# lrjconan/LanczosNetwork

Measured on NVIDIA H100. Metric: QM8 molecules/sec (forward), higher is better.
Workload: dtype f32

## Files before the change

### lanczosnetwork_b200/csrc/filter_mlp_chain.cu

```cuda
#include "tc_gemm.cuh"

namespace {

constexpr int S0MAX = 8;

struct ChainPolicy {
  static constexpr int kStagesB = 2;
  static constexpr int kStagesA = 4;
  struct Params {
    const float* table;
    const int32_t* rowmap;
    const int32_t* nrows;
    const float* W_hi;
    const float* W_lo;
    const float* bias_all;
    float* coeff;
    int Rall, L, S, Hd;
    int dbg;
  };
  static __device__ __forceinline__ bool mma0(const Params& p) { return p.S > S0MAX; }
  static __device__ __forceinline__ int first_stage(const Params& p) { return mma0(p) ? 0 : 1; }
  static __device__ __forceinline__ int steps_per_item(const Params& p) { return mma0(p) ? 4 : 2; }
  static __device__ __forceinline__ int rows(const Params& p) { return p.nrows ? __ldg(p.nrows) : p.Rall; }
  static __device__ __forceinline__ int ntile(const Params& p) { return (rows(p) + tcg::BM - 1) / tcg::BM; }
  static __device__ __forceinline__ void item_range(const Params& p, int cta, int ncta, int& first,
                                                    int& count) {
    const int items = ntile(p) * p.L, base = items / ncta, rem = items % ncta;
    count = base + (cta < rem ? 1 : 0);
    first = cta * base + min(cta, rem);
  }
  static __device__ __forceinline__ int num_steps(const Params& p, int cta, int ncta) {
    int first, count;
    item_range(p, cta, ncta, first, count);
    return count * steps_per_item(p);
  }
  static __device__ __forceinline__ void decode(const Params& p, int cta, int ncta, int it,
                                                int& m_tile, int& sub) {
    const int per = steps_per_item(p), nt = ntile(p);
    int first, count;
    item_range(p, cta, ncta, first, count);
    const int item = first + it / per;
    m_tile = item % nt;
    sub = (item / nt) * 4 + first_stage(p) + it % per;
  }
  static __device__ __forceinline__ int num_kblocks(const Params& p, int sub) {
    return (sub & 3) == 0 ? 1 : p.Hd / tcg::BK;
  }
  static __device__ __forceinline__ int w_row0(const Params& p, int layer, int stage) {
    return layer * (3 * p.Hd + p.S) + stage * p.Hd;
  }
  static __device__ __forceinline__ void w_coords(const Params& p, int sub, int kb, int& col0, int& row0) {
    col0 = kb * tcg::BK;
    row0 = w_row0(p, sub >> 2, sub & 3);
  }
  static __device__ __forceinline__ bool operand_from_acc(const Params& p, int sub) {
    return (sub & 3) > first_stage(p);
  }
  static __device__ __forceinline__ float acc_operand(const Params&, const uint8_t* policy_smem, int sub, int col,
                                                      float x) {
    const float* bs = reinterpret_cast<const float*>(policy_smem) + BS_OFF;
    return fmaxf(x + bs[(sub & 3) * tcg::BN + col], 0.f);
  }

  const Params& p;
  const int tid, r;
  static constexpr int BS_OFF = 2 * tcg::BN * S0MAX;
  float* W1s;
  float* W3s;
  float* bs;
  float* b3s;
  int src, cur_layer;
  float tv[S0MAX];
  float o[S0MAX];

  static size_t smem_bytes() {
    return (BS_OFF + 3 * tcg::BN + S0MAX) * 4;
  }

  __device__ ChainPolicy(const Params& p_, uint8_t* smem, int tid_)
      : p(p_), tid(tid_), r(tid_ & 127), src(-1), cur_layer(-1) {
    W1s = reinterpret_cast<float*>(smem);
    W3s = W1s + tcg::BN * S0MAX;
    bs = W1s + BS_OFF;
    b3s = bs + 3 * tcg::BN;
  }

  __device__ void step_begin(int m_tile, int sub, int, tcg::PhaseTimer& tm) {
    const int layer = sub >> 2;
    if ((sub & 3) != first_stage(p)) return;
    const int i = m_tile * tcg::BM + r;
    src = i < rows(p) ? (p.rowmap ? __ldg(p.rowmap + i) : i) : -1;
    if (layer != cur_layer) {
      tcg::producers_sync<ChainPolicy>();
      const int row0 = w_row0(p, layer, 0), row3 = w_row0(p, layer, 3);
      if (!mma0(p)) {
#pragma unroll 4
        for (int e = tid; e < p.Hd * S0MAX; e += tcg::producer_threads<ChainPolicy>) {
          const int c = e / S0MAX, k = e - c * S0MAX;
          const int64_t o1 = (int64_t)(row0 + c) * p.Hd + k;
          W1s[e] = (k < p.S) ? __ldg(p.W_hi + o1) + __ldg(p.W_lo + o1) : 0.f;
          const int64_t o3 = (int64_t)(row3 + k) * p.Hd + c;
          W3s[e] = (k < p.S) ? __ldg(p.W_hi + o3) + __ldg(p.W_lo + o3) : 0.f;
        }
        if (tid < S0MAX) b3s[tid] = tid < p.S ? __ldg(p.bias_all + row3 + tid) : 0.f;
      }
      for (int e = tid; e < 3 * tcg::BN; e += tcg::producer_threads<ChainPolicy>) {
        const int st = e / tcg::BN, c = e - st * tcg::BN;
        bs[e] = c < p.Hd ? __ldg(p.bias_all + row0 + st * p.Hd + c) : 0.f;
      }
      tcg::producers_sync<ChainPolicy>();
      cur_layer = layer;
      tm.lap(1);
    }
    if (mma0(p)) return;
#pragma unroll
    for (int k = 0; k < S0MAX; ++k)
      tv[k] = (src >= 0 && k < p.S) ? __ldg(p.table + (int64_t)src * p.S + k) : 0.f;
  }

  __device__ __forceinline__ void produce(int sub, int kb, float (&v)[32]) {
    if ((sub & 3) == 0) {
#pragma unroll
      for (int j = 0; j < 32; ++j)
        v[j] = (src >= 0 && j < p.S) ? __ldg(p.table + (int64_t)src * p.S + j) : 0.f;
      return;
    }
#pragma unroll
    for (int j = 0; j < 32; ++j) {
      const int c = kb * tcg::BK + j;
      const float4* wr = reinterpret_cast<const float4*>(W1s + c * S0MAX);
      const float4 wa = wr[0], wb = wr[1];
      float a = bs[c];
      a = fmaf(tv[0], wa.x, a); a = fmaf(tv[1], wa.y, a); a = fmaf(tv[2], wa.z, a); a = fmaf(tv[3], wa.w, a);
      a = fmaf(tv[4], wb.x, a); a = fmaf(tv[5], wb.y, a); a = fmaf(tv[6], wb.z, a); a = fmaf(tv[7], wb.w, a);
      v[j] = fmaxf(a, 0.f);
    }
  }
  __device__ __forceinline__ void pre_epilogue(int) {}
  __device__ __forceinline__ void post_epilogue(int) {}

  __device__ __forceinline__ void store(int sub, int col, const float (&x)[tcg::EW]) {
    const int layer = sub >> 2, stage = sub & 3;
    if (stage == 3) {
      if (src < 0 || col >= p.S) return;
      const float* bias = p.bias_all + w_row0(p, layer, stage);
      float* dst = p.coeff + ((int64_t)layer * p.Rall + src) * p.S;
#pragma unroll
      for (int j = 0; j < tcg::EW; ++j)
        if (col + j < p.S) dst[col + j] = x[j] + __ldg(bias + col + j);
      return;
    }
    if (col >= p.Hd) return;
    const float* b2 = bs + 2 * tcg::BN;
    if (col == 0) {
#pragma unroll
      for (int s = 0; s < S0MAX; ++s) o[s] = 0.f;
    }
#pragma unroll
    for (int j = 0; j < tcg::EW; ++j) {
      const float y = fmaxf(x[j] + b2[col + j], 0.f);
      const float4* wr = reinterpret_cast<const float4*>(W3s + (col + j) * S0MAX);
      const float4 wa = wr[0], wb = wr[1];
      o[0] = fmaf(y, wa.x, o[0]); o[1] = fmaf(y, wa.y, o[1]);
      o[2] = fmaf(y, wa.z, o[2]); o[3] = fmaf(y, wa.w, o[3]);
      o[4] = fmaf(y, wb.x, o[4]); o[5] = fmaf(y, wb.y, o[5]);
      o[6] = fmaf(y, wb.z, o[6]); o[7] = fmaf(y, wb.w, o[7]);
    }
    if (col + tcg::EW < p.Hd || src < 0) return;
    float* dst = p.coeff + ((int64_t)layer * p.Rall + src) * p.S;
#pragma unroll
    for (int s = 0; s < S0MAX; ++s)
      if (s < p.S) dst[s] = o[s] + b3s[s];
  }
};

__global__ void __launch_bounds__(1024)
ritz_rowmap_kernel(const int32_t* __restrict__ gext, int B, int K, int32_t* __restrict__ rowmap,
                   int32_t* __restrict__ nrows) {
  __shared__ int warp_sums[32];
  __shared__ int gbase[1024], gk[1024];
  __shared__ int running;
  const int tid = threadIdx.x, lane = tid & 31, warp = tid >> 5;
  if (tid == 0) running = 0;
  __syncthreads();
  for (int b0 = 0; b0 < B; b0 += 1024) {
    const int b = b0 + tid;
    int k = (b < B) ? min(gext[b * 2 + 1], K) : 0;
    int incl = k;
#pragma unroll
    for (int o = 1; o < 32; o <<= 1) {
      const int t = __shfl_up_sync(0xffffffffu, incl, o);
      if (lane >= o) incl += t;
    }
    if (lane == 31) warp_sums[warp] = incl;
    __syncthreads();
    if (warp == 0) {
      int w = warp_sums[lane], wi = w;
#pragma unroll
      for (int o = 1; o < 32; o <<= 1) {
        const int t = __shfl_up_sync(0xffffffffu, wi, o);
        if (lane >= o) wi += t;
      }
      warp_sums[lane] = wi - w;
    }
    __syncthreads();
    const int base = running + warp_sums[warp] + incl - k;
    gbase[tid] = base;
    gk[tid] = k;
    __syncthreads();
    if (tid == 1023) running = base + k;
    for (int j = warp; j < 1024 && b0 + j < B; j += 32)
      for (int i = lane; i < gk[j]; i += 32) rowmap[gbase[j] + i] = (b0 + j) * K + i;
    __syncthreads();
  }
  if (tid == 0) nrows[0] = running;
}

}

extern "C" {

int lnb_ritz_rowmap(lnb_stream_t stream, const int32_t* gext, int B, int K, int32_t* rowmap,
                    int32_t* nrows) {
  LNB_REQUIRE(gext && rowmap && nrows, "ritz_rowmap: null pointer");
  LNB_REQUIRE(B >= 0 && K >= 1, "ritz_rowmap: bad dims");
  ritz_rowmap_kernel<<<1, 1024, 0, (cudaStream_t)stream>>>(gext, B, K, rowmap, nrows);
  lnb::count_launch();
  return lnb::finish_launch("ritz_rowmap");
}

int lnb_ritz_filter_mlp(lnb_stream_t stream, const float* table, const int32_t* rowmap,
                        const int32_t* nrows, const float* W_hi, const float* W_lo,
                        const float* bias_all, int Rall, int L, int S, int Hd, float* coeff) {
  return lnb_ritz_filter_mlp_ctas(stream, table, rowmap, nrows, W_hi, W_lo, bias_all, Rall, L, S, Hd,
                                  coeff, 0);
}

int lnb_ritz_filter_mlp_ctas(lnb_stream_t stream, const float* table, const int32_t* rowmap,
                             const int32_t* nrows, const float* W_hi, const float* W_lo,
                             const float* bias_all, int Rall, int L, int S, int Hd, float* coeff,
                             int ctas) {
  LNB_REQUIRE(table && W_hi && W_lo && bias_all && coeff, "ritz_filter_mlp: null pointer");
  LNB_REQUIRE((rowmap == nullptr) == (nrows == nullptr), "ritz_filter_mlp: rowmap and nrows go together");
  LNB_REQUIRE(Rall >= 0 && L >= 1 && S >= 1 && Hd >= 1 && ctas >= 0, "ritz_filter_mlp: bad dims");
  if (S > 32 || Hd % 32 != 0 || Hd > tcg::BN) {
    lnb::set_err("ritz_filter_mlp: unsupported shape S=%d hidden=%d (needs S<=32, hidden%%32==0, hidden<=128)", S, Hd);
    return LNB_ERR_UNSUPPORTED;
  }
  if (Rall == 0) return LNB_OK;
  const size_t smem = tcg::core_smem(ChainPolicy::kStagesB, ChainPolicy::kStagesA) + 1024 + ChainPolicy::smem_bytes();
  ChainPolicy::Params p{table, rowmap, nrows, W_hi, W_lo, bias_all, coeff, Rall, L, S, Hd, tcg::debug_flags()};
  return tcg::launch<ChainPolicy>(stream, W_hi, W_lo, L * (3 * Hd + S), Hd, smem, lnb::ceil_div(Rall, tcg::BM) * L, p,
                                  "ritz_filter_mlp", ctas);
}

}
```

### lanczosnetwork_b200/csrc/tc_gemm.cuh

```cuda
#pragma once
#include "common.cuh"
#include "sm90.cuh"
#include <stdlib.h>
#include <type_traits>
#include <utility>

namespace tcg {

constexpr int BM = 128, BN = 128, BK = 32;
constexpr int TILE_B_BYTES = BN * BK * 4;
constexpr int STAGE_B_BYTES = 2 * TILE_B_BYTES;
constexpr int TILE_A_BYTES = BM * BK * 4;
constexpr int STAGE_A_BYTES = 2 * TILE_A_BYTES;
constexpr int EW = 16;
constexpr int CONSUMER_THREADS = 256;
constexpr int CONSUMER_REGS = 168;
constexpr int MAX_B_STAGES = 6, MAX_A_STAGES = 4;

template <class P, class = void> struct ProducerGroups : std::integral_constant<int, 1> {};
template <class P>
struct ProducerGroups<P, std::void_t<decltype(P::kProducerGroups)>> : std::integral_constant<int, P::kProducerGroups> {};
template <class P> constexpr int producer_threads = 128 * ProducerGroups<P>::value;
template <class P> constexpr int cta_threads = producer_threads<P> + CONSUMER_THREADS;
template <class P> constexpr int producer_regs = (65536 - CONSUMER_THREADS * CONSUMER_REGS) / producer_threads<P> / 8 * 8;
__host__ __device__ constexpr int core_smem(int stages_b, int stages_a) {
  return stages_b * STAGE_B_BYTES + stages_a * STAGE_A_BYTES + 256;
}
__host__ __device__ constexpr int pass_cols(int stages_a) {
  return stages_a * STAGE_A_BYTES / (BM * 4) < BN ? stages_a * STAGE_A_BYTES / (BM * 4) : BN;
}

__device__ __forceinline__ uint8_t* a_ring(uint8_t* policy_smem, int stages_b, int stages_a) {
  return policy_smem - core_smem(stages_b, stages_a) + stages_b * STAGE_B_BYTES;
}

struct Core {
  uint8_t* Bst;
  uint8_t* Ast;
  uint64_t* b_full;
  uint64_t* b_empty;
  uint64_t* a_full;
  uint64_t* a_empty;
  uint64_t* stg_full;
  uint64_t* stg_empty;
  uint64_t* kept_read;
};

__device__ __forceinline__ Core carve(uint8_t* base, int stages_b, int stages_a) {
  Core c;
  c.Bst = base;
  c.Ast = base + stages_b * STAGE_B_BYTES;
  uint64_t* bars = reinterpret_cast<uint64_t*>(c.Ast + stages_a * STAGE_A_BYTES);
  c.b_full = bars;
  c.b_empty = c.b_full + MAX_B_STAGES;
  c.a_full = c.b_empty + MAX_B_STAGES;
  c.a_empty = c.a_full + MAX_A_STAGES;
  c.stg_full = c.a_empty + MAX_A_STAGES;
  c.stg_empty = c.stg_full + 1;
  c.kept_read = c.stg_empty + 1;
  return c;
}

__device__ unsigned long long* g_prof = nullptr;

struct PhaseTimer {
  unsigned long long* buf;
  long long t0;
  __device__ __forceinline__ void start(int cta, int tid) {
    buf = (tid == 0 && g_prof) ? g_prof + cta * 32 : nullptr;
    if (buf) t0 = clock64();
  }
  __device__ __forceinline__ void start_if(int cta, bool owner) {
    buf = (owner && g_prof) ? g_prof + cta * 32 : nullptr;
    if (buf) t0 = clock64();
  }
  __device__ __forceinline__ void lap(int slot) {
    if (buf) { long long t = clock64(); atomicAdd(&buf[slot], (unsigned long long)(t - t0)); t0 = t; }
  }
};

template <class Policy>
__device__ __forceinline__ void producers_sync() {
  asm volatile("bar.sync 1, %0;" ::"n"(producer_threads<Policy>) : "memory");
}
__device__ __forceinline__ void consumers_sync() {
  asm volatile("bar.sync 2, %0;" ::"n"(CONSUMER_THREADS) : "memory");
}

__device__ __forceinline__ int stg_index(int row, int col, int pw) {
  return row * pw + ((((col >> 2) ^ row) & (pw / 4 - 1)) << 2) + (col & 3);
}

template <class P, class = void> struct HasAccInit : std::false_type {};
template <class P> struct HasAccInit<P, std::void_t<decltype(&P::acc_init)>> : std::true_type {};
template <class P, class = void> struct HasOperandFromAcc : std::false_type {};
template <class P> struct HasOperandFromAcc<P, std::void_t<decltype(&P::operand_from_acc)>> : std::true_type {};
template <class P>
constexpr bool kScaledProduce =
    std::is_same_v<decltype(std::declval<P&>().produce(0, 0, std::declval<float (&)[32]>())), float>;

template <class Policy>
__device__ __forceinline__ bool next_from_acc(const typename Policy::Params& p, int cta, int ncta, int it,
                                              int nsteps, int& nkb_next) {
  if (it + 1 >= nsteps) return false;
  int m_tile, sub;
  Policy::decode(p, cta, ncta, it + 1, m_tile, sub);
  nkb_next = Policy::num_kblocks(p, sub);
  return Policy::operand_from_acc(p, sub);
}

constexpr int SKIP_MMA = 2;
constexpr int SKIP_TMA = 4;

template <class Policy, int kSkip>
__device__ __forceinline__ void tc_gemm_body(const CUtensorMap& map_hi, const CUtensorMap& map_lo,
                                             const typename Policy::Params& p) {
  extern __shared__ __align__(16) uint8_t smem_raw[];
  const uint32_t pad = (1024u - (sm90::smem_u32(smem_raw) & 1023u)) & 1023u;
  uint8_t* base = smem_raw + pad;
  constexpr int SB = Policy::kStagesB, SA = Policy::kStagesA;
  static_assert(SB >= 1 && SB <= MAX_B_STAGES && SA >= 1 && SA <= MAX_A_STAGES, "ring depths");
  constexpr int PW = pass_cols(SA);
  constexpr int NPASS = BN / PW;
  constexpr bool kAccInit = HasAccInit<Policy>::value;
  static_assert(!kAccInit || NPASS == 1, "a drain kept in the A ring must fit it in one pass");
  constexpr bool kOpAcc = HasOperandFromAcc<Policy>::value;
  constexpr bool kQueue = !kAccInit;
  static_assert(!kOpAcc || SA * BK >= BN, "an operand written from the accumulators needs one A stage per k-block");
  constexpr int NG = ProducerGroups<Policy>::value, PT = producer_threads<Policy>;
  constexpr bool kScaled = kScaledProduce<Policy>;
  static_assert(NG == 1 || (NG == 2 && !kOpAcc && PW % (2 * EW) == 0), "two producer groups: no operand_from_acc");
  Core c = carve(base, SB, SA);
  uint8_t* policy_smem = base + core_smem(SB, SA);
  float* stg = reinterpret_cast<float*>(c.Ast);

  const int tid = threadIdx.x, warp = tid >> 5, lane = tid & 31;
  const int role = __shfl_sync(0xffffffffu, tid / 128, 0);
  const int cta = blockIdx.x, ncta = gridDim.x;
  const int nsteps = __shfl_sync(0xffffffffu, Policy::num_steps(p, cta, ncta), 0);
  unsigned long long prof_ns0 = 0;
  long long prof_c0 = 0;
  if (tid == 0 && g_prof) {
    asm volatile("mov.u64 %0, %globaltimer;" : "=l"(prof_ns0));
    prof_c0 = clock64();
  }

  if (warp == PT / 32 && lane == 0) {
    sm90::tma_prefetch_desc(&map_hi);
    sm90::tma_prefetch_desc(&map_lo);
    for (int s = 0; s < SB; ++s) {
      sm90::mbar_init(&c.b_full[s], 1);
      sm90::mbar_init(&c.b_empty[s], CONSUMER_THREADS / 32);
    }
    for (int s = 0; s < SA; ++s) {
      sm90::mbar_init(&c.a_full[s], PT / NG);
      sm90::mbar_init(&c.a_empty[s], CONSUMER_THREADS / 32);
    }
    sm90::mbar_init(c.stg_full, CONSUMER_THREADS);
    sm90::mbar_init(c.stg_empty, PT);
    sm90::mbar_init(c.kept_read, CONSUMER_THREADS / 32);
    sm90::fence_barrier_init();
  }
  __syncthreads();

  if (NG == 1 ? role == 0 : role < NG) {
    if constexpr (NG > 1) sm90::setmaxnreg_dec<producer_regs<Policy>>();
    const int r = tid & 127;
    const int grp = NG == 1 ? 0 : role;
    Policy pol(p, policy_smem, tid);
    uint32_t cnt = 0;
    uint32_t npass = 0;
    uint32_t nkept = 0;
    bool after_kept = false;
    for (int it = 0; it < nsteps; ++it) {
      int m_tile, sub;
      Policy::decode(p, cta, ncta, it, m_tile, sub);
      int nkb = Policy::num_kblocks(p, sub);
      bool kept = false, to_acc = false;
      if constexpr (kAccInit) kept = Policy::drain_kept(p, sub);
      if constexpr (kOpAcc) {
        if (Policy::operand_from_acc(p, sub)) nkb = 0;
        int nkb_next;
        to_acc = next_from_acc<Policy>(p, cta, ncta, it, nsteps, nkb_next);
      }
      PhaseTimer tm;
      tm.start(cta, tid);
      pol.step_begin(m_tile, sub, NG == 1 ? 0 : (int)((grp + NG - cnt % NG) % NG), tm);
      [[maybe_unused]] float v_kept[32];
      for (int kb = 0; kb < nkb; ++kb, ++cnt) {
        if constexpr (NG > 1) {
          if (cnt % NG != (uint32_t)grp) continue;
        }
        float v[32];
        [[maybe_unused]] float scale = 1.f;
        if (!(p.dbg & 8)) {
          if constexpr (kScaled) scale = pol.produce(sub, kb, v_kept);
          else pol.produce(sub, kb, v);
        }
        const uint32_t sa = cnt % SA;
        if (kAccInit && (NG == 1 ? kb == 0 : kb < NG) && after_kept) {
          sm90::mbar_wait(c.kept_read, nkept & 1u);
          if constexpr (NG == 1) ++nkept;
        }
        sm90::mbar_wait(&c.a_empty[sa], ((cnt / SA) & 1u) ^ 1u);
        if (!(p.dbg & 1)) {
          uint8_t* hi = c.Ast + sa * STAGE_A_BYTES + r * 128;
#pragma unroll
          for (int j = 0; j < 8; ++j) {
            if constexpr (kScaled) {
#pragma unroll
              for (int i = 4 * j; i < 4 * j + 4; ++i) v[i] = __fmul_rn(scale, v_kept[i]);
            }
            uint4 h, l;
            h.x = sm90::tf32_rna_bits(v[4 * j + 0]); h.y = sm90::tf32_rna_bits(v[4 * j + 1]);
            h.z = sm90::tf32_rna_bits(v[4 * j + 2]); h.w = sm90::tf32_rna_bits(v[4 * j + 3]);
            l.x = sm90::tf32_rna_bits(v[4 * j + 0] - __uint_as_float(h.x));
            l.y = sm90::tf32_rna_bits(v[4 * j + 1] - __uint_as_float(h.y));
            l.z = sm90::tf32_rna_bits(v[4 * j + 2] - __uint_as_float(h.z));
            l.w = sm90::tf32_rna_bits(v[4 * j + 3] - __uint_as_float(h.w));
            const int off = (j ^ (r & 7)) * 16;
            *reinterpret_cast<uint4*>(hi + off) = h;
            *reinterpret_cast<uint4*>(hi + TILE_A_BYTES + off) = l;
          }
        }
        sm90::fence_proxy_async();
        sm90::mbar_arrive(&c.a_full[sa]);
      }
      if constexpr (NG > 1) {
        if (kAccInit && after_kept) ++nkept;
      }
      tm.lap((sub & 1) ? 8 : 3);
      pol.pre_epilogue(sub);
      tm.lap(4);
#pragma unroll 1
      for (int q = 0; q < (kept || to_acc ? 0 : NPASS); ++q, ++npass) {
        sm90::mbar_wait(c.stg_full, npass & 1u);
        if (q == 0) tm.lap((sub & 1) ? 9 : 5);
#pragma unroll 1
        for (int col = q * PW + grp * EW; col < (q + 1) * PW; col += NG * EW) {
          float x[EW];
#pragma unroll
          for (int j = 0; j < EW; j += 4) {
            const float4 t = *reinterpret_cast<const float4*>(stg + stg_index(r, col - q * PW + j, PW));
            x[j] = t.x; x[j + 1] = t.y; x[j + 2] = t.z; x[j + 3] = t.w;
          }
          pol.store(sub, col, x);
        }
        sm90::mbar_arrive(c.stg_empty);
      }
      tm.lap(7);
      producers_sync<Policy>();
      pol.post_epilogue(sub);
      tm.lap(10);
      after_kept = kept;
    }
  } else {
    if constexpr (NG > 1) sm90::setmaxnreg_inc<CONSUMER_REGS>();
    const int wg = role - NG;
    const int wq = warp & 3;
    float d[128];
    uint32_t cnt = 0, npass = 0;
    uint32_t nacc = 0;
    bool after_kept = false;
    const int row0 = wg * 64 + wq * 16 + (lane >> 2), cl = 2 * (lane & 3);
    const bool w_issuer = warp == PT / 32;
    int l_it = 0, l_kb = 0, l_nkb = -1, l_sub = 0;
    uint32_t l_cnt = 0;
    auto load_next = [&]() {
      while (l_it < nsteps) {
        if (l_nkb < 0) {
          int mt;
          Policy::decode(p, cta, ncta, l_it, mt, l_sub);
          l_nkb = Policy::num_kblocks(p, l_sub);
        }
        if (l_kb < l_nkb) break;
        ++l_it; l_kb = 0; l_nkb = -1;
      }
      if (l_it >= nsteps) return;
      int col0, row0;
      Policy::w_coords(p, l_sub, l_kb, col0, row0);
      const uint32_t st = l_cnt % SB;
      sm90::mbar_wait_uniform(&c.b_empty[st], ((l_cnt / SB) & 1u) ^ 1u);
      uint8_t* dst = c.Bst + st * STAGE_B_BYTES;
      sm90::tma_load_2d_pair_elected<(kSkip & SKIP_TMA) != 0>(w_issuer, &c.b_full[st], STAGE_B_BYTES, dst, &map_hi,
                                                               dst + TILE_B_BYTES, &map_lo, col0, row0);
      ++l_kb; ++l_cnt;
    };
    auto release = [&](uint32_t sb_rel, bool a_stage, uint32_t sa_rel) {
      sm90::mbar_arrive_pred(&c.a_empty[sa_rel], a_stage && lane == 0);
      sm90::mbar_arrive_pred(&c.b_empty[sb_rel], lane == 0);
      load_next();
    };
    for (int i = 0; i < SB; ++i) load_next();
    for (int it = 0; it < nsteps; ++it) {
      int m_tile, sub;
      Policy::decode(p, cta, ncta, it, m_tile, sub);
      const int nkb = Policy::num_kblocks(p, sub);
      bool kept = false, from_acc = false, to_acc = false;
      int nkb_next = 0;
      if constexpr (kOpAcc) {
        from_acc = Policy::operand_from_acc(p, sub);
        to_acc = next_from_acc<Policy>(p, cta, ncta, it, nsteps, nkb_next);
      }
      if constexpr (kAccInit) {
        kept = Policy::drain_kept(p, sub);
        sm90::wgmma_fence_operand(d);
        if (!Policy::acc_init(p, policy_smem, stg, sub, row0, cl, d)) {
#pragma unroll
          for (int i = 0; i < 128; ++i) d[i] = 0.f;
        }
        if (after_kept) {
          __syncwarp();
          if (lane == 0) sm90::mbar_arrive(c.kept_read);
        }
      } else {
#pragma unroll
        for (int i = 0; i < 128; ++i) d[i] = 0.f;
      }
      sm90::wgmma_fence_operand(d);
      for (int kb = 0; kb < nkb; ++kb, ++cnt) {
        const uint32_t acnt = cnt - nacc;
        const uint32_t sb = cnt % SB, sa = from_acc ? (uint32_t)kb : acnt % SA;
        sm90::mbar_wait_uniform(&c.b_full[sb], (cnt / SB) & 1u);
        if (!from_acc) sm90::mbar_wait_uniform(&c.a_full[sa], (acnt / SA) & 1u);
        if constexpr (!(kSkip & SKIP_MMA)) {
          const uint32_t a_hi = sm90::smem_u32(c.Ast + sa * STAGE_A_BYTES) + wg * 64 * 128;
          const uint32_t a_lo = a_hi + TILE_A_BYTES;
          const uint32_t b = sm90::smem_u32(c.Bst + sb * STAGE_B_BYTES);
          sm90::wgmma_fence_operand(d);
          sm90::wgmma_fence();
#pragma unroll
          for (int k = 0; k < BK / 8; ++k) {
            const uint64_t ah = sm90::wgmma_desc_kmajor_sw128(a_hi + 32 * k);
            const uint64_t wh = sm90::wgmma_desc_kmajor_sw128(b + 32 * k);
            sm90::wgmma_n128(d, ah, wh, 1u);
            sm90::wgmma_n128_hi(d, ah, sm90::wgmma_desc_kmajor_sw128(b + TILE_B_BYTES + 32 * k), 1u);
            sm90::wgmma_n128_hi(d, sm90::wgmma_desc_kmajor_sw128(a_lo + 32 * k), wh, 1u);
          }
          sm90::wgmma_commit();
          if constexpr (kQueue) sm90::wgmma_wait_one();
          else sm90::wgmma_wait_all();
          sm90::wgmma_fence_operand(d);
        }
        if constexpr (kQueue) {
          if (kb > 0) release((cnt - 1) % SB, !from_acc, from_acc ? (uint32_t)(kb - 1) : (acnt - 1) % SA);
        } else {
          release(sb, !from_acc, sa);
        }
      }
      if constexpr (!(kSkip & SKIP_MMA)) {
        sm90::wgmma_wait_all();
        sm90::wgmma_fence_operand(d);
      }
      if (kQueue && nkb > 0)
        release((cnt - 1) % SB, !from_acc, from_acc ? (uint32_t)(nkb - 1) : (cnt - nacc - 1) % SA);
      if (from_acc) nacc += nkb;
      PhaseTimer ctm;
      if (to_acc) ctm.start_if(cta, tid == PT);
      consumers_sync();
      if (to_acc) {
        if constexpr (kOpAcc) {
#pragma unroll
          for (int i = 0; i < 64; i += 2) {
            const int col = 8 * (i / 4) + cl, row = row0 + 8 * ((i / 2) % 2), kb = i / 16;
            if (kb < nkb_next) {
              const float y0 = Policy::acc_operand(p, policy_smem, sub, col, d[i] + d[i + 64]);
              const float y1 = Policy::acc_operand(p, policy_smem, sub, col + 1, d[i + 1] + d[i + 65]);
              uint2 h, l;
              h.x = sm90::tf32_rna_bits(y0); h.y = sm90::tf32_rna_bits(y1);
              l.x = sm90::tf32_rna_bits(y0 - __uint_as_float(h.x));
              l.y = sm90::tf32_rna_bits(y1 - __uint_as_float(h.y));
              uint8_t* dst = c.Ast + kb * STAGE_A_BYTES + row * 128 + (((((col & 31) >> 2) ^ row) & 7) << 4) +
                             (col & 3) * 4;
              *reinterpret_cast<uint2*>(dst) = h;
              *reinterpret_cast<uint2*>(dst + TILE_A_BYTES) = l;
            }
          }
          sm90::fence_proxy_async();
          consumers_sync();
          ctm.lap(14);
        }
      } else {
#pragma unroll
        for (int q = 0; q < NPASS; ++q, npass += kept ? 0 : 1) {
          if (!kept) sm90::mbar_wait(c.stg_empty, (npass & 1u) ^ 1u);
#pragma unroll
          for (int i = 0; i < 64; i += 2) {
            const int col = 8 * (i / 4) + cl, row = row0 + 8 * ((i / 2) % 2);
            if (col >= q * PW && col < (q + 1) * PW)
              *reinterpret_cast<float2*>(stg + stg_index(row, col - q * PW, PW)) =
                  make_float2(d[i] + d[i + 64], d[i + 1] + d[i + 65]);
          }
          if (!kept) sm90::mbar_arrive(c.stg_full);
        }
      }
      if (kept) consumers_sync();
      after_kept = kept;
    }
  }

  __syncthreads();
  if (tid == 0 && g_prof) {
    unsigned long long ns1;
    asm volatile("mov.u64 %0, %globaltimer;" : "=l"(ns1));
    atomicAdd(&g_prof[cta * 32 + 11], ns1 - prof_ns0);
    atomicAdd(&g_prof[cta * 32 + 12], (unsigned long long)(clock64() - prof_c0));
    g_prof[cta * 32 + 13] = prof_ns0;
  }
}

template <class Policy>
__global__ void __launch_bounds__(cta_threads<Policy>, 1)
tc_gemm_kernel(const __grid_constant__ CUtensorMap map_hi,
               const __grid_constant__ CUtensorMap map_lo, const typename Policy::Params p) {
  tc_gemm_body<Policy, 0>(map_hi, map_lo, p);
}

template <class Policy, int kSkip>
__global__ void __launch_bounds__(cta_threads<Policy>, 1)
tc_gemm_probe_kernel(const __grid_constant__ CUtensorMap map_hi,
                     const __grid_constant__ CUtensorMap map_lo, const typename Policy::Params p) {
  tc_gemm_body<Policy, kSkip>(map_hi, map_lo, p);
}

__device__ __forceinline__ void store_row_chunk(float* orow, int ncols, const float* bias, bool relu,
                                                int col, const float (&x)[EW]) {
  if (orow == nullptr || col >= ncols) return;
  const bool vec_ok = (reinterpret_cast<uintptr_t>(orow + col) & 15) == 0;
#pragma unroll
  for (int j = 0; j < EW; j += 4) {
    float o[4];
#pragma unroll
    for (int u = 0; u < 4; ++u) {
      const int n = col + j + u;
      float y = x[j + u];
      if (n < ncols) {
        if (bias) y += __ldg(bias + n);
        if (relu) y = fmaxf(y, 0.f);
      }
      o[u] = y;
    }
    if (vec_ok && col + j + 3 < ncols) {
      *reinterpret_cast<float4*>(orow + col + j) = make_float4(o[0], o[1], o[2], o[3]);
    } else {
#pragma unroll
      for (int u = 0; u < 4; ++u)
        if (col + j + u < ncols) orow[col + j + u] = o[u];
    }
  }
}

typedef CUresult (*EncodeTiledFn)(CUtensorMap*, CUtensorMapDataType, cuuint32_t, void*,
                                  const cuuint64_t*, const cuuint64_t*, const cuuint32_t*,
                                  const cuuint32_t*, CUtensorMapInterleave, CUtensorMapSwizzle,
                                  CUtensorMapL2promotion, CUtensorMapFloatOOBfill);

inline EncodeTiledFn get_encode_fn() {
  static EncodeTiledFn fn = nullptr;
  if (!fn) {
    void* ptr = nullptr;
    cudaDriverEntryPointQueryResult q;
    if (cudaGetDriverEntryPoint("cuTensorMapEncodeTiled", &ptr, cudaEnableDefault, &q) == cudaSuccess &&
        q == cudaDriverEntryPointSuccess)
      fn = reinterpret_cast<EncodeTiledFn>(ptr);
  }
  return fn;
}

inline int make_weight_map(CUtensorMap* map, const float* W, int rows, int cols, const char* who,
                           int box_rows = BN) {
  EncodeTiledFn enc = get_encode_fn();
  if (!enc) { lnb::set_err("%s: cuTensorMapEncodeTiled unavailable", who); return LNB_ERR_UNSUPPORTED; }
  cuuint64_t gdim[2] = {(cuuint64_t)cols, (cuuint64_t)rows};
  cuuint64_t gstride[1] = {(cuuint64_t)cols * sizeof(float)};
  cuuint32_t box[2] = {(cuuint32_t)BK, (cuuint32_t)box_rows};
  cuuint32_t estr[2] = {1, 1};
  CUresult r = enc(map, CU_TENSOR_MAP_DATA_TYPE_FLOAT32, 2, const_cast<float*>(W), gdim, gstride,
                   box, estr, CU_TENSOR_MAP_INTERLEAVE_NONE, CU_TENSOR_MAP_SWIZZLE_128B,
                   CU_TENSOR_MAP_L2_PROMOTION_L2_256B, CU_TENSOR_MAP_FLOAT_OOB_FILL_NONE);
  if (r != CUDA_SUCCESS) {
    lnb::set_err("%s: cuTensorMapEncodeTiled failed (CUresult %d)", who, (int)r);
    return LNB_ERR_ARG;
  }
  return LNB_OK;
}

inline int debug_flags() {
  const char* e = getenv("LNB_DBG");
  return e ? atoi(e) : 0;
}

inline int sm_count() {
  int dev = 0, n = 132;
  if (cudaGetDevice(&dev) == cudaSuccess)
    cudaDeviceGetAttribute(&n, cudaDevAttrMultiProcessorCount, dev);
  return n > 0 ? n : 132;
}

static unsigned long long* g_prof_mirrored = nullptr;

static int sync_prof_buffer(const char* who) {
  unsigned long long* buf = lnb::prof_buffer();
  if (buf == g_prof_mirrored) return LNB_OK;
  cudaError_t e = cudaMemcpyToSymbol(g_prof, &buf, sizeof(buf));
  if (e != cudaSuccess) { lnb::set_err("%s: %s", who, cudaGetErrorString(e)); return (int)e; }
  g_prof_mirrored = buf;
  return LNB_OK;
}

template <class Pol>
static int launch(lnb_stream_t stream, const float* W_hi, const float* W_lo, int w_rows, int w_cols,
                  size_t smem, int items, const typename Pol::Params& p, const char* who,
                  int max_ctas = 0) {
  CUtensorMap map_hi, map_lo;
  int rc = make_weight_map(&map_hi, W_hi, w_rows, w_cols, who);
  if (rc != LNB_OK) return rc;
  rc = make_weight_map(&map_lo, W_lo, w_rows, w_cols, who);
  if (rc != LNB_OK) return rc;
  rc = sync_prof_buffer(who);
  if (rc != LNB_OK) return rc;
  const int skip = p.dbg & (SKIP_MMA | SKIP_TMA);
  auto kern = skip == 0                    ? tc_gemm_kernel<Pol>
              : skip == SKIP_MMA           ? tc_gemm_probe_kernel<Pol, SKIP_MMA>
              : skip == SKIP_TMA           ? tc_gemm_probe_kernel<Pol, SKIP_TMA>
                                           : tc_gemm_probe_kernel<Pol, SKIP_MMA | SKIP_TMA>;
  cudaFuncSetAttribute(kern, cudaFuncAttributeMaxDynamicSharedMemorySize, (int)smem);
  int grid = items < sm_count() ? items : sm_count();
  if (max_ctas > 0 && grid > max_ctas) grid = max_ctas;
  kern<<<grid, cta_threads<Pol>, smem, (cudaStream_t)stream>>>(map_hi, map_lo, p);
  lnb::count_launch();
  return lnb::finish_launch(who);
}

}
```

Before: 1.180 million.

## Let producers prefetch next chain stage's A operand while epilogue drains

Reserves the first A-ring stages as a separate drain area by moving the epilogue staging buffer up, and lets producers begin the next step within the same layer (step_begin plus producing its first k-blocks into the reserved stages) before draining the current accumulator. A new acc_free barrier tells producers when the consumer has finished reading from-accumulator stages. The output row is latched in pre_epilogue so the early step_begin cannot overwrite it. The goal is to overlap A-operand production with the epilogue, at the cost of a smaller staging pass width and more complex barrier phase tracking.

```diff
diff --git a/lanczosnetwork_b200/csrc/filter_mlp_chain.cu b/lanczosnetwork_b200/csrc/filter_mlp_chain.cu
--- a/lanczosnetwork_b200/csrc/filter_mlp_chain.cu
+++ b/lanczosnetwork_b200/csrc/filter_mlp_chain.cu
@@ -7,6 +7,7 @@
 struct ChainPolicy {
   static constexpr int kStagesB = 2;
   static constexpr int kStagesA = 4;
+  static constexpr int kDrainStage = 2;
   struct Params {
     const float* table;
     const int32_t* rowmap;
@@ -56,6 +57,9 @@
   static __device__ __forceinline__ bool operand_from_acc(const Params& p, int sub) {
     return (sub & 3) > first_stage(p);
   }
+  static __device__ __forceinline__ bool lead(const Params& p, int sub, int sub_next) {
+    return !mma0(p) && (sub_next >> 2) == (sub >> 2);
+  }
   static __device__ __forceinline__ float acc_operand(const Params&, const uint8_t* policy_smem, int sub, int col,
                                                       float x) {
     const float* bs = reinterpret_cast<const float*>(policy_smem) + BS_OFF;
@@ -70,6 +74,7 @@
   float* bs;
   float* b3s;
   int src, cur_layer;
+  int out_row;
   float tv[S0MAX];
   float o[S0MAX];
 
@@ -78,7 +83,7 @@
   }
 
   __device__ ChainPolicy(const Params& p_, uint8_t* smem, int tid_)
-      : p(p_), tid(tid_), r(tid_ & 127), src(-1), cur_layer(-1) {
+      : p(p_), tid(tid_), r(tid_ & 127), src(-1), cur_layer(-1), out_row(-1) {
     W1s = reinterpret_cast<float*>(smem);
     W3s = W1s + tcg::BN * S0MAX;
     bs = W1s + BS_OFF;
@@ -136,15 +141,15 @@
       v[j] = fmaxf(a, 0.f);
     }
   }
-  __device__ __forceinline__ void pre_epilogue(int) {}
+  __device__ __forceinline__ void pre_epilogue(int) { out_row = src; }
   __device__ __forceinline__ void post_epilogue(int) {}
 
   __device__ __forceinline__ void store(int sub, int col, const float (&x)[tcg::EW]) {
     const int layer = sub >> 2, stage = sub & 3;
     if (stage == 3) {
-      if (src < 0 || col >= p.S) return;
+      if (out_row < 0 || col >= p.S) return;
       const float* bias = p.bias_all + w_row0(p, layer, stage);
-      float* dst = p.coeff + ((int64_t)layer * p.Rall + src) * p.S;
+      float* dst = p.coeff + ((int64_t)layer * p.Rall + out_row) * p.S;
 #pragma unroll
       for (int j = 0; j < tcg::EW; ++j)
         if (col + j < p.S) dst[col + j] = x[j] + __ldg(bias + col + j);
@@ -166,8 +171,8 @@
       o[4] = fmaf(y, wb.x, o[4]); o[5] = fmaf(y, wb.y, o[5]);
       o[6] = fmaf(y, wb.z, o[6]); o[7] = fmaf(y, wb.w, o[7]);
     }
-    if (col + tcg::EW < p.Hd || src < 0) return;
-    float* dst = p.coeff + ((int64_t)layer * p.Rall + src) * p.S;
+    if (col + tcg::EW < p.Hd || out_row < 0) return;
+    float* dst = p.coeff + ((int64_t)layer * p.Rall + out_row) * p.S;
 #pragma unroll
     for (int s = 0; s < S0MAX; ++s)
       if (s < p.S) dst[s] = o[s] + b3s[s];
diff --git a/lanczosnetwork_b200/csrc/tc_gemm.cuh b/lanczosnetwork_b200/csrc/tc_gemm.cuh
--- a/lanczosnetwork_b200/csrc/tc_gemm.cuh
+++ b/lanczosnetwork_b200/csrc/tc_gemm.cuh
@@ -21,6 +21,9 @@
 template <class P>
 struct ProducerGroups<P, std::void_t<decltype(P::kProducerGroups)>> : std::integral_constant<int, P::kProducerGroups> {};
 template <class P> constexpr int producer_threads = 128 * ProducerGroups<P>::value;
+template <class P, class = void> struct DrainStage : std::integral_constant<int, 0> {};
+template <class P>
+struct DrainStage<P, std::void_t<decltype(P::kDrainStage)>> : std::integral_constant<int, P::kDrainStage> {};
 template <class P> constexpr int cta_threads = producer_threads<P> + CONSUMER_THREADS;
 template <class P> constexpr int producer_regs = (65536 - CONSUMER_THREADS * CONSUMER_REGS) / producer_threads<P> / 8 * 8;
 __host__ __device__ constexpr int core_smem(int stages_b, int stages_a) {
@@ -44,6 +47,7 @@
   uint64_t* stg_full;
   uint64_t* stg_empty;
   uint64_t* kept_read;
+  uint64_t* acc_free;
 };
 
 __device__ __forceinline__ Core carve(uint8_t* base, int stages_b, int stages_a) {
@@ -58,6 +62,7 @@
   c.stg_full = c.a_empty + MAX_A_STAGES;
   c.stg_empty = c.stg_full + 1;
   c.kept_read = c.stg_empty + 1;
+  c.acc_free = c.kept_read + 1;
   return c;
 }
 
@@ -95,6 +100,25 @@
 template <class P> struct HasAccInit<P, std::void_t<decltype(&P::acc_init)>> : std::true_type {};
 template <class P, class = void> struct HasOperandFromAcc : std::false_type {};
 template <class P> struct HasOperandFromAcc<P, std::void_t<decltype(&P::operand_from_acc)>> : std::true_type {};
+template <class P, class = void> struct HasLead : std::false_type {};
+template <class P> struct HasLead<P, std::void_t<decltype(&P::lead)>> : std::true_type {};
+
+__device__ __forceinline__ void put_row_split(uint8_t* stage, int r, const float (&v)[32]) {
+  uint8_t* hi = stage + r * 128;
+#pragma unroll
+  for (int j = 0; j < 8; ++j) {
+    uint4 h, l;
+    h.x = sm90::tf32_rna_bits(v[4 * j + 0]); h.y = sm90::tf32_rna_bits(v[4 * j + 1]);
+    h.z = sm90::tf32_rna_bits(v[4 * j + 2]); h.w = sm90::tf32_rna_bits(v[4 * j + 3]);
+    l.x = sm90::tf32_rna_bits(v[4 * j + 0] - __uint_as_float(h.x));
+    l.y = sm90::tf32_rna_bits(v[4 * j + 1] - __uint_as_float(h.y));
+    l.z = sm90::tf32_rna_bits(v[4 * j + 2] - __uint_as_float(h.z));
+    l.w = sm90::tf32_rna_bits(v[4 * j + 3] - __uint_as_float(h.w));
+    const int off = (j ^ (r & 7)) * 16;
+    *reinterpret_cast<uint4*>(hi + off) = h;
+    *reinterpret_cast<uint4*>(hi + TILE_A_BYTES + off) = l;
+  }
+}
 template <class P>
 constexpr bool kScaledProduce =
     std::is_same_v<decltype(std::declval<P&>().produce(0, 0, std::declval<float (&)[32]>())), float>;
@@ -120,7 +144,9 @@
   uint8_t* base = smem_raw + pad;
   constexpr int SB = Policy::kStagesB, SA = Policy::kStagesA;
   static_assert(SB >= 1 && SB <= MAX_B_STAGES && SA >= 1 && SA <= MAX_A_STAGES, "ring depths");
-  constexpr int PW = pass_cols(SA);
+  constexpr int DS = DrainStage<Policy>::value;
+  static_assert(DS >= 0 && DS < SA, "drain stage");
+  constexpr int PW = pass_cols(SA - DS);
   constexpr int NPASS = BN / PW;
   constexpr bool kAccInit = HasAccInit<Policy>::value;
   static_assert(!kAccInit || NPASS == 1, "a drain kept in the A ring must fit it in one pass");
@@ -130,9 +156,12 @@
   constexpr int NG = ProducerGroups<Policy>::value, PT = producer_threads<Policy>;
   constexpr bool kScaled = kScaledProduce<Policy>;
   static_assert(NG == 1 || (NG == 2 && !kOpAcc && PW % (2 * EW) == 0), "two producer groups: no operand_from_acc");
+  constexpr bool kLead = HasLead<Policy>::value;
+  static_assert(!kLead || (kOpAcc && DS > 0 && NPASS == 1 && NG == 1 && !kScaled), "lead(): see the contract");
+  static_assert(kLead || DS == 0, "kDrainStage goes with lead()");
   Core c = carve(base, SB, SA);
   uint8_t* policy_smem = base + core_smem(SB, SA);
-  float* stg = reinterpret_cast<float*>(c.Ast);
+  float* stg = reinterpret_cast<float*>(c.Ast + DS * STAGE_A_BYTES);
 
   const int tid = threadIdx.x, warp = tid >> 5, lane = tid & 31;
   const int role = __shfl_sync(0xffffffffu, tid / 128, 0);
@@ -159,6 +188,9 @@
     sm90::mbar_init(c.stg_full, CONSUMER_THREADS);
     sm90::mbar_init(c.stg_empty, PT);
     sm90::mbar_init(c.kept_read, CONSUMER_THREADS / 32);
+    if constexpr (kLead) {
+      for (int s = 0; s < DS; ++s) sm90::mbar_init(&c.acc_free[s], CONSUMER_THREADS / 32);
+    }
     sm90::fence_barrier_init();
   }
   __syncthreads();
@@ -172,10 +204,14 @@
     uint32_t npass = 0;
     uint32_t nkept = 0;
     bool after_kept = false;
+    [[maybe_unused]] int led = 0;
+    [[maybe_unused]] bool begun = false;
+    [[maybe_unused]] uint32_t acc_steps[DS > 0 ? DS : 1] = {};
     for (int it = 0; it < nsteps; ++it) {
       int m_tile, sub;
       Policy::decode(p, cta, ncta, it, m_tile, sub);
       int nkb = Policy::num_kblocks(p, sub);
+      [[maybe_unused]] const int nkb_mma = nkb;
       bool kept = false, to_acc = false;
       if constexpr (kAccInit) kept = Policy::drain_kept(p, sub);
       if constexpr (kOpAcc) {
@@ -183,11 +219,25 @@
         int nkb_next;
         to_acc = next_from_acc<Policy>(p, cta, ncta, it, nsteps, nkb_next);
       }
+      if constexpr (kLead) {
+        if (nkb == 0) {
+#pragma unroll
+          for (int s = 0; s < DS; ++s) acc_steps[s] += s < nkb_mma ? 1u : 0u;
+        }
+      }
       PhaseTimer tm;
       tm.start(cta, tid);
-      pol.step_begin(m_tile, sub, NG == 1 ? 0 : (int)((grp + NG - cnt % NG) % NG), tm);
+      int kb0 = 0;
+      bool began = false;
+      if constexpr (kLead) {
+        kb0 = led;
+        began = begun;
+        led = 0;
+        begun = false;
+      }
+      if (!began) pol.step_begin(m_tile, sub, NG == 1 ? 0 : (int)((grp + NG - cnt % NG) % NG), tm);
       [[maybe_unused]] float v_kept[32];
-      for (int kb = 0; kb < nkb; ++kb, ++cnt) {
+      for (int kb = kb0; kb < nkb; ++kb, ++cnt) {
         if constexpr (NG > 1) {
           if (cnt % NG != (uint32_t)grp) continue;
         }
@@ -232,6 +282,31 @@
       tm.lap((sub & 1) ? 8 : 3);
       pol.pre_epilogue(sub);
       tm.lap(4);
+      if constexpr (kLead) {
+        if (nkb == 0 && !to_acc && it + 1 < nsteps) {
+          int m_next, sub_next;
+          Policy::decode(p, cta, ncta, it + 1, m_next, sub_next);
+          if (Policy::lead(p, sub, sub_next) && !Policy::operand_from_acc(p, sub_next)) {
+            const int nkb_next = Policy::num_kblocks(p, sub_next);
+            pol.step_begin(m_next, sub_next, 0, tm);
+            begun = true;
+            for (led = 0; led < nkb_next && cnt % SA < (uint32_t)DS; ++led, ++cnt) {
+              float v[32];
+              if (!(p.dbg & 8)) pol.produce(sub_next, led, v);
+              const uint32_t sa = cnt % SA;
+              uint32_t used = 0;
+#pragma unroll
+              for (int s = 0; s < DS; ++s) used = (uint32_t)s == sa ? acc_steps[s] : used;
+              if ((int)sa < nkb_mma) sm90::mbar_wait(&c.acc_free[sa], (used - 1) & 1u);
+              sm90::mbar_wait(&c.a_empty[sa], ((cnt / SA) & 1u) ^ 1u);
+              if (!(p.dbg & 1)) put_row_split(c.Ast + sa * STAGE_A_BYTES, r, v);
+              sm90::fence_proxy_async();
+              sm90::mbar_arrive(&c.a_full[sa]);
+            }
+          }
+        }
+        tm.lap(6);
+      }
 #pragma unroll 1
       for (int q = 0; q < (kept || to_acc ? 0 : NPASS); ++q, ++npass) {
         sm90::mbar_wait(c.stg_full, npass & 1u);
@@ -288,6 +363,8 @@
     };
     auto release = [&](uint32_t sb_rel, bool a_stage, uint32_t sa_rel) {
       sm90::mbar_arrive_pred(&c.a_empty[sa_rel], a_stage && lane == 0);
+      if constexpr (kLead)
+        sm90::mbar_arrive_pred(&c.acc_free[sa_rel % MAX_A_STAGES], !a_stage && sa_rel < (uint32_t)DS && lane == 0);
       sm90::mbar_arrive_pred(&c.b_empty[sb_rel], lane == 0);
       load_next();
     };
```

After: 1.184 million (median of 6 runs). No clear change (+0.3%).
